# SMART-TTS/SMART-NAR_Fast_TTS

Measured on AMD Instinct MI355X. Metric: mel_frames_per_sec, higher is better.
Workload: dtype f32

## Files before the change

### include/nar_fs2.h

```cpp
#ifndef NAR_FS2_H
#define NAR_FS2_H

#include <stddef.h>
#include <stdint.h>

#ifdef __cplusplus
extern "C" {
#endif

#define NS_ABI_VERSION 6

typedef struct ns_model ns_model;

typedef struct ns_config {
  int32_t n_vocab;
  int32_t max_seq_len;
  int32_t d_enc, n_enc_layer, n_enc_head;
  int32_t d_dec, n_dec_layer, n_dec_head;
  int32_t d_inner;
  int32_t ffn_k1, ffn_k2;
  int32_t vp_filter, vp_kernel;
  int32_t n_bins;
  int32_t n_mel;
  int32_t postnet_dim, postnet_k, postnet_n;
// ... 37 lines not shown
                                 size_t ws_aln_bytes, float* log_d, uint8_t* src_mask, int64_t* mel_lens, float* p_pred, float* e_pred,
                                 float* tgt_output, float* attn_all_layers, int64_t* d_targets, void* stream);
int ns_upload_lengths(const int64_t* host, int n, int64_t* dev, void* stream);

#define NS_STATUS_TRUNCATED 1
#define NS_STATUS_BAD_TOKEN 2
int ns_forward_mel(ns_model* m, int B, int L, int T, const int64_t* mel_lens, float p_control, float e_control,
                   const float* p_targets, const float* e_targets, const void* ws_enc, void* ws_dec, size_t ws_dec_bytes,
                   float* mel, float* postnet_mel, float* p_pred, float* e_pred, uint8_t* mel_mask, int32_t* status, void* stream);

int ns_forward_mel_packed(ns_model* m, int B, int L, int T, const int64_t* mel_lens, const int64_t* mel_lens_host,
                          float p_control, float e_control, const float* p_targets, const float* e_targets, const void* ws_enc,
                          void* ws_dec, size_t ws_dec_bytes, float* mel, float* postnet_mel, float* p_pred, float* e_pred,
                          uint8_t* mel_mask, int32_t* status, void* stream);
int64_t ns_last_phase2_rows(const ns_model* m);

size_t ns_op_ws_bytes(const ns_model* m, int B, int S);
int ns_op_mask_from_lengths(const int64_t* lens, int B, int max_len, uint8_t* mask, void* stream);
int ns_op_sinusoid_table(int n_position, int d_hid, float* out, void* stream);
int ns_op_txt_encoder(ns_model* m, const int64_t* texts, const int64_t* lens, int B, int L, float* out, void* ws, size_t ws_bytes, void* stream);
int ns_op_multi_head_attention(ns_model* m, const char* prefix, const float* x, const int64_t* lens, int B, int S, float* out, void* ws, size_t ws_bytes, void* stream);
int ns_op_positionwise_ffn(ns_model* m, const char* prefix, const float* x, int B, int S, float* out, void* ws, size_t ws_bytes, void* stream);
int ns_op_fft_block(ns_model* m, const char* prefix, const float* x, const int64_t* lens, int B, int S, float* out, void* ws, size_t ws_bytes, void* stream);
int ns_op_variance_predictor(ns_model* m, const char* prefix, const float* x, const int64_t* lens, int B, int S, float* out, void* ws, size_t ws_bytes, void* stream);
int ns_op_predictor_conv1(ns_model* m, const char* prefix, const float* x, int B, int S, float* h, void* ws, size_t ws_bytes, void* stream);
int ns_op_predictor_tail(ns_model* m, const char* prefix, const float* h, const int64_t* lens, int B, int S, float control,
                         const float* target , const float* x_in , int add_pos, float* pred,
                         float* x_out , void* ws, size_t ws_bytes, void* stream);
int ns_op_duration_round(const float* log_d, int n, float d_control, float* d_rounded, void* stream);
int ns_op_duration_scan(const float* d_rounded, int B, int L, int32_t* cum, int64_t* mel_lens, void* stream);
// ... 312 lines not shown
```

### smart-nar_fast_tts_amd/_lib.py

```python
from __future__ import annotations

import ctypes as C
import os

import torch

_HERE = os.path.dirname(os.path.abspath(__file__))
LIB_PATH = os.path.join(_HERE, "csrc", "libnarfs2.so")


class NsConfig(C.Structure):
    _fields_ = [(n, C.c_int32) for n in (
        "n_vocab", "max_seq_len", "d_enc", "n_enc_layer", "n_enc_head", "d_dec", "n_dec_layer", "n_dec_head",
        "d_inner", "ffn_k1", "ffn_k2", "vp_filter", "vp_kernel", "n_bins", "n_mel",
        "postnet_dim", "postnet_k", "postnet_n", "pitch_frame_level", "energy_frame_level", "length_regulator",
        "matmul_bf16x3", "row_epilogue", "phase1_packing")]


class NsLossArgs(C.Structure):
    _fields_ = ([(n, C.c_int32) for n in ("B", "L", "T", "H", "n_mel", "pitch_frame_level", "energy_frame_level")]
                + [(n, C.c_int64) for n in ("mel_targets_stride", "d_targets_stride")]
                + [(n, C.c_void_p) for n in ("mel", "postnet", "mel_targets", "mel_masks", "pitch", "pitch_targets", "energy", "energy_targets",
                                             "log_d", "d_targets", "src_masks", "src_lens", "mel_lens")]
                + [("attn", C.c_void_p * 4)])
# ... 39 lines not shown
class NsPgWeights(C.Structure):
    _fields_ = [(n, C.c_void_p) for n in PG_NAMES]


class NsPgGrads(C.Structure):
    _fields_ = [(n, C.c_void_p) for n in PG_NAMES + ("dx",)]


class NsMelConfig(C.Structure):
    _fields_ = [(n, C.c_int32) for n in ("filter_length", "hop_length", "win_length", "n_mel")] + [("clip_val", C.c_float)]


class NsGlConfig(C.Structure):
    _fields_ = [(n, C.c_int32) for n in ("filter_length", "hop_length", "win_length", "n_mel")] + [("spec_from_mel_scaling", C.c_float)]


_P, _I, _F, _Z, _S = C.c_void_p, C.c_int, C.c_float, C.c_size_t, C.c_char_p

SIGNATURES = {
    "ns_last_error": (C.c_char_p, []),
    "ns_create": (_I, [C.POINTER(NsConfig), C.POINTER(_P)]),
    "ns_destroy": (None, [_P]),
    "ns_arena_bytes": (_Z, [_P]),
    "ns_bind_arena": (_I, [_P, _P, _Z]),
    "ns_set_weight": (_I, [_P, _S, _P, C.POINTER(C.c_int64), _I]),
    "ns_check_weight": (_I, [_P, _S, C.POINTER(C.c_int64), _I]),
    "ns_finalize_weights": (_I, [_P, _P]),
    "ns_adopt_arena": (_I, [_P]),
    "ns_encoder_ws_bytes": (_Z, [_P, _I, _I]),
    "ns_decoder_ws_bytes": (_Z, [_P, _I, _I, _I]),
    "ns_forward_durations": (_I, [_P, _P, _P, _I, _I, _F, _F, _F, _P, _P, _P, _Z, _P, _P, _P, _P, _P, _P, _P, _P]),
    "ns_forward_durations_packed": (_I, [_P, _P, _P, _P, _I, _I, _F, _F, _F, _P, _P, _P, _Z, _P, _P, _P, _P, _P, _P, _P, _P]),
    "ns_forward_durations_teacher": (_I, [_P, _P, _P, _P, _P, _P, _I, _I, _I, _F, _F, _P, _P, _P, _Z, _P, _Z, _P, _P, _P, _P, _P, _P, _P, _P, _P]),
    "ns_last_phase1_rows": (C.c_int64, [_P]),
    "ns_upload_lengths": (_I, [_P, _I, _P, _P]),
    "ns_forward_mel": (_I, [_P, _I, _I, _I, _P, _F, _F, _P, _P, _P, _P, _Z, _P, _P, _P, _P, _P, _P, _P]),
    "ns_forward_mel_packed": (_I, [_P, _I, _I, _I, _P, _P, _F, _F, _P, _P, _P, _P, _Z, _P, _P, _P, _P, _P, _P, _P]),

    "ns_last_phase2_rows": (C.c_int64, [_P]),
    "ns_plan_gemm": (_I, [_I, _I, _I, _I, C.POINTER(C.c_int32)]),
    "ns_plan_gemm_launches": (_I, [_I, _I, _I, _I, _I, C.POINTER(C.c_int32)]),
    "ns_plan_row_tile": (_I, [_I, _I]),
    "ns_plan_row_tile_k": (_I, [_I, _I, _I]),
    "ns_acc_chunk": (_I, []),
    "ns_abi_version": (_I, []),
    "ns_plan_attention_split": (_I, [_I, _I, _I, _I]),
    "ns_op_ws_bytes": (_Z, [_P, _I, _I]),
    "ns_op_mask_from_lengths": (_I, [_P, _I, _I, _P, _P]),
    "ns_op_sinusoid_table": (_I, [_I, _I, _P, _P]),
    "ns_op_txt_encoder": (_I, [_P, _P, _P, _I, _I, _P, _P, _Z, _P]),
    "ns_op_multi_head_attention": (_I, [_P, _S, _P, _P, _I, _I, _P, _P, _Z, _P]),
    "ns_op_positionwise_ffn": (_I, [_P, _S, _P, _I, _I, _P, _P, _Z, _P]),
    "ns_op_fft_block": (_I, [_P, _S, _P, _P, _I, _I, _P, _P, _Z, _P]),
    "ns_op_variance_predictor": (_I, [_P, _S, _P, _P, _I, _I, _P, _P, _Z, _P]),
# ... 166 lines not shown
```

### smart-nar_fast_tts_amd/csrc/api.hip

```cpp
#include <cstdio>

#include "../../include/nar_fs2.h"
#include "host_core.h"

using namespace ns;

static thread_local std::string g_err;
static int fail(const std::string& s) { g_err = s; return 1; }

namespace {

struct LayerW { ConvW qkv, fc, w1, w2; size_t ln1_g, ln1_b, ln2_g, ln2_b; };
struct PredW { ConvW c1, c2; size_t ln1_g, ln1_b, ln2_g, ln2_b, lin_w, lin_b; };

}

struct ns_model {
  ns_config cfg;
  std::vector<LayerW> enc, dec;
  PredW pred[3];
  size_t hdr;
  size_t emb, enc_pos, dec_pos, pitch_bins, energy_bins, pitch_emb, energy_emb;
  ConvW mel_linear;
  size_t pn_in, pn_hid, pn_const;
  size_t pos_long;
  std::vector<ConvW> post;
  Arena ar;
  float* arena = nullptr;
  bool ready = false;
  WeightRegistry weights;
  const float* P(size_t off) const { return arena + off; }
  const unsigned short* plane(size_t off) const { return off != NO_PLANE ? reinterpret_cast<const unsigned short*>(P(off)) : nullptr; }
  ConvGemm conv(const ConvW& w) const {
// ... 151 lines not shown
    ConvW w = m->ar.conv(cout, c.postnet_k, cin);
    if (c.matmul_bf16x3 == 1 && cin == c.postnet_dim && cout == c.postnet_dim) take_b3(m->ar, w);
    if (c.matmul_bf16x3 == 2) take_bf(m->ar, w);
    m->post.push_back(w);
  }
  m->pn_in = m->ar.take((size_t)PN_CONST_ROWS * c.n_mel);
  m->pn_hid = m->ar.take((size_t)2 * PN_CONST_ROWS * c.postnet_dim);
  m->pn_const = m->ar.take((size_t)PN_CONST_ROWS * c.n_mel);
  m->pos_long = m->ar.take((size_t)POS_LONG_ROWS * c.d_dec);
  *out = m;
  return 0;
}

extern "C" void ns_destroy(ns_model* m) {
  if (!m) return;
  for (auto& ps : m->prof_slot)
    for (auto& ev : ps.ev) { (void)hipEventDestroy(ev.first); (void)hipEventDestroy(ev.second); }
  delete m;
}
extern "C" size_t ns_arena_bytes(const ns_model* m) { return m ? m->ar.n * sizeof(float) : 0; }

extern "C" int ns_bind_arena(ns_model* m, void* dev, size_t bytes) { return bind_arena(m, dev, bytes, ns_arena_bytes(m), "ns_bind_arena"); }

extern "C" int ns_adopt_arena(ns_model* m) {
  if (!m || !m->arena) return fail("ns_adopt_arena: no arena bound");
  uint32_t got[ARENA_HDR_WORDS], want[ARENA_HDR_WORDS];
  int cur_dev = 0;
  NS_HIP(hipGetDevice(&cur_dev));
  hipPointerAttribute_t at;
  NS_HIP(hipPointerGetAttributes(&at, m->arena));
// ... 103 lines not shown
  NS_HIP(launch_sinusoid(POS_LONG_ROWS, c.d_dec, m->arena + m->pos_long, st));
  NS_HIP(hipStreamSynchronize(st));
  m->weights.release();
  m->ready = true;
  return 0;
}

namespace {
struct PackedCtx { RowMap rm; int Mp; };

struct Scratch {
  const PackedCtx* pk;
  float *xa, *xb, *qkv, *att, *t1, *x1, *hid, *vp1, *vp2, *pos_ext, *att_part;
  size_t att_part_floats;
  Tickets tk;
};

static size_t imax(size_t a, size_t b) { return a > b ? a : b; }

static Scratch carve(const ns_config& c, Bump& bp, size_t M, int S, bool no_split = false) {
  Scratch s;
  s.pk = nullptr;
  const size_t d = c.d_enc;
  s.xa = bp.f(M * d); s.xb = bp.f(M * d);
  s.qkv = bp.f(M * 3 * d); s.att = bp.f(M * d); s.t1 = bp.f(M * d); s.x1 = bp.f(M * d);
  s.hid = bp.f(M * imax(c.d_inner, 2 * (size_t)c.postnet_dim));
  s.vp1 = bp.f(M * c.vp_filter); s.vp2 = bp.f(M * c.vp_filter);
  s.pos_ext = S > c.max_seq_len ? bp.f((size_t)S * d) : nullptr;
  const int hmax = c.n_enc_head > c.n_dec_head ? c.n_enc_head : c.n_dec_head;
  int nsp = 1;
// ... 244 lines not shown
  sc.hid = m->arena + m->pn_hid;
  return postnet(m, in, 1, PN_CONST_ROWS, in, m->arena + m->pn_const, sc, st);
}

static int encoder(ns_model* m, const long long* texts, const long long* lens, int B, int L, float* out, Scratch& sc,
                   hipStream_t st) {
  const ns_config& c = m->cfg;
  const int M = rows_of(sc, B, L), d = c.d_enc;
  const float* pos;
  NS_TRY(position_rows(m, m->enc_pos, L, d, sc, &pos, st));
  float* cur = m->enc.empty() ? out : sc.xa;
  if (sc.pk) NS_HIP(launch_embed_pos_packed(texts, m->P(m->emb), pos, cur, sc.pk->rm, B, M, L, d, c.n_vocab, sc.tk.base, TICKET_INTS, st));
  else NS_HIP(launch_embed_pos(texts, m->P(m->emb), pos, cur, M, L, d, c.n_vocab, sc.tk.base, TICKET_INTS, st));
  for (size_t i = 0; i < m->enc.size(); ++i) {
    float* dst = (i + 1 == m->enc.size()) ? out : (cur == sc.xa ? sc.xb : sc.xa);
    NS_TRY(fft_block(m, m->enc[i], d, c.n_enc_head, cur, lens, B, L, dst, sc, st));
    cur = dst;
  }
  return 0;
}

static int decoder_stack(ns_model* m, float* x, const long long* lens, int B, int T, float* out, Scratch& sc, hipStream_t st) {
  const ns_config& c = m->cfg;
  float* cur = x;
  float* alt = (x == sc.xa) ? sc.xb : sc.xa;
  for (size_t i = 0; i < m->dec.size(); ++i) {
    float* dst = (i + 1 == m->dec.size()) ? out : alt;
    NS_TRY(fft_block(m, m->dec[i], c.d_dec, c.n_dec_head, cur, lens, B, T, dst, sc, st));
    if (dst != out) { alt = cur; cur = dst; }
  }
// ... 30 lines not shown
  ns_aligner* aln;
  const float* mels;
  const int64_t* mel_lens_in;
  int T;
  void* ws_aln;
  size_t ws_aln_bytes;
  float *tgt_output, *attn;
  int64_t* d_targets;
};

static int forward_durations(ns_model* m, const int64_t* texts, const int64_t* src_lens, const int64_t* lens_host, int B, int L, float d_control,
                             float p_control, float e_control, const float* p_targets, const float* e_targets,
                             void* ws_enc, size_t ws_bytes, float* log_d, float* d_rounded, uint8_t* src_mask,
                             int64_t* mel_lens, float* p_pred, float* e_pred, int64_t* mel_lens_host, void* stream,
                             const Teacher* tf = nullptr) {
  NS_TRY(check_ready(m));
  if (B <= 0 || L <= 0) return fail("ns_forward_durations: empty batch");
  if (ws_bytes < ns_encoder_ws_bytes(m, B, L)) return fail("ns_forward_durations: workspace too small");
  hipStream_t st = (hipStream_t)stream;
  const ns_config& c = m->cfg;
  if (!c.pitch_frame_level && !p_pred) return fail("ns_forward_durations: phoneme_level pitch needs a p_pred [B,L] output");
  if (!c.energy_frame_level && !e_pred) return fail("ns_forward_durations: phoneme_level energy needs an e_pred [B,L] output");
  Bump bp(ws_enc);
  float* enc_out = bp.f((size_t)B * L * c.d_enc);
  int32_t* cum = (int32_t*)bp.raw((size_t)B * L * sizeof(int32_t));
  float* dur_keep = bp.f((size_t)B * L);
  const long long* lens = (const long long*)src_lens;
  size_t Mp = 0;
  bool packed = lens_host && !m->enc.empty() && launch_planner_enabled() && c.pitch_frame_level && c.energy_frame_level && c.phase1_packing != 2;
  if (packed) {
    Mp = phase1_packed_rows(lens_host, B, L);
    auto cu_rows = [&](size_t rows) {
      const size_t ntn = (size_t)c.d_inner / 128, w32 = (rows + 31) / 32 * ntn, w48 = (rows + 47) / 48 * ntn;
      return (conv_gemm_tile16_enabled() && w32 > 256 && w48 <= 256) ? (size_t)48 : 32 * ((w32 + 255) / 256);
    };
    packed = Mp > 0 && Mp * 10 <= (size_t)B * L * 9 && (c.phase1_packing == 1 || cu_rows(Mp) < cu_rows((size_t)B * L));
  }
  const size_t Mrows = packed ? Mp : (size_t)B * L;
  m->last_rows1 = (long long)Mrows;
  Scratch sc = carve(c, bp, Mrows, L, packed);
  PackedCtx pk;
  memset(&pk, 0, sizeof(pk));
  float *enc_w = enc_out, *logd_w = log_d;
  if (packed) {
    const int M = (int)Mp, d = c.d_enc;
    const int base = window_att_wgs(lens_host, B, L, PHONEME_GUARD, c.n_enc_head);
    size_t n = (size_t)attention_split_packed(base, L, d / c.n_enc_head, Mp, d);
    const size_t per = Mp * d + 2 * Mp * c.n_enc_head;
    const size_t extra = phase1_packed_extra_bytes(c, B, L);
    const size_t avail = ws_bytes > bp.off + extra ? (ws_bytes - bp.off - extra) / sizeof(float) : 0;
    while (n > 1 && n * per > avail) --n;
    if (n > 1) { sc.att_part_floats = n * per; sc.att_part = bp.f(sc.att_part_floats); }
    int* plan = (int*)bp.raw(pack_plan_ints(B, Mp) * sizeof(int));
    enc_w = bp.f(Mp * d); logd_w = bp.f(Mp);
    if (bp.off > ws_bytes) return fail("ns_forward_durations: workspace too small (packed rows)");
    pk.Mp = M;
    pk.rm.rows = M;
    pk.rm.att_wgs = base;
    NS_HIP(launch_pack_plan_only(lens, B, L, c.n_enc_head, M, plan, &pk.rm, st, PHONEME_GUARD));
  }
  {
    sc.pk = packed ? &pk : nullptr;
    NS_TRY(encoder(m, (const long long*)texts, lens, B, L, enc_w, sc, st));
    if (tf) {
      if (tf->T > 0) NS_TRY(ns_aln_forward(tf->aln, enc_w, src_lens, tf->mels, tf->mel_lens_in, B, L, tf->T, tf->tgt_output, tf->attn, tf->d_targets,
                                           tf->ws_aln, tf->ws_aln_bytes, stream));
      else NS_HIP(hipMemsetAsync(tf->d_targets, 0, (size_t)B * L * sizeof(int64_t), st));
    }
    NS_TRY(predictor(m, m->pred[0], enc_w, lens, B, L, 1.0f, nullptr, logd_w, nullptr, nullptr, nullptr, nullptr, sc, st));
    if (!c.pitch_frame_level)
      NS_TRY(predictor(m, m->pred[1], enc_w, lens, B, L, p_control, p_targets, p_pred, m->P(m->pitch_bins), m->P(m->pitch_emb), nullptr, enc_w, sc, st));
    if (!c.energy_frame_level)
      NS_TRY(predictor(m, m->pred[2], enc_w, lens, B, L, e_control, e_targets, e_pred, m->P(m->energy_bins), m->P(m->energy_emb), nullptr, enc_w, sc, st));
  }
  if (packed) {
    NS_HIP(launch_unpack_phase1(pk.rm, lens, B, L, c.d_enc, enc_w, enc_out, logd_w, log_d, st));
  }
  if (tf) {
    NS_HIP(launch_duration_target_tail((const long long*)tf->d_targets, lens, (const long long*)texts, c.n_vocab, B, L, dur_keep, cum,
                                       (long long*)mel_lens, src_mask, st));
    return 0;
  }
  NS_HIP(launch_duration_tail(log_d, lens, (const long long*)texts, c.n_vocab, B, L, d_control, d_rounded, dur_keep, cum,
// ... 115 lines not shown
      NS_HIP(launch_pack_plan(lens, B, T, c.n_dec_head, M, plan, &pk.rm, st));
      NS_HIP(launch_gaussian_upsampling(enc_out, dur_keep, B, L, c.d_enc, T, T, sc.xa, sc.vp2, nullptr, lens, status, sc.tk.base, TICKET_INTS, st, &pk.rm));
    } else {
      NS_HIP(launch_length_regulate_packed(enc_out, cum, B, L, c.d_enc, T, M, c.n_dec_head, sc.xa, lens, status, sc.tk.base, TICKET_INTS, plan, &pk.rm, st));
    }
    pk.rm.att_wgs = window_att_wgs(lens_host, B, T, PACK_GUARD, c.n_dec_head);
    if (p_targets && c.pitch_frame_level) { NS_HIP(launch_pack_vector(pk.rm, T, p_targets, pt_p, M, st)); p_targets = pt_p; }
    if (e_targets && c.energy_frame_level) { NS_HIP(launch_pack_vector(pk.rm, T, e_targets, et_p, M, st)); e_targets = et_p; }
  } else if (c.length_regulator == 1) {
    NS_HIP(launch_mask_from_lengths(lens, B, T, mel_mask, st));
    if ((size_t)B * (L + 1) > (size_t)M * c.vp_filter) return fail("ns_forward_mel: workspace too small for the Gaussian centres");
    NS_HIP(launch_gaussian_upsampling(enc_out, dur_keep, B, L, c.d_enc, T, T, sc.xa, sc.vp2, nullptr, lens, status, sc.tk.base, TICKET_INTS, st));
  } else {
    NS_HIP(launch_length_regulate(enc_out, cum, B, L, c.d_enc, T, sc.xa, mel_mask, lens, status, sc.tk.base, TICKET_INTS, st));
  }
  sc.pk = packed ? &pk : nullptr;
  float* const mel_dst = packed ? mel_p : mel;
  float* const post_dst = packed ? post_p : postnet_mel;
  float* const pp_dst = packed ? pp_p : p_pred;
  float* const ep_dst = packed ? ep_p : e_pred;
  const float* pos;
  NS_TRY(position_rows(m, m->dec_pos, T, d, sc, &pos, st));
  float* cur = sc.xa;
  float* alt = sc.xb;
  if (c.pitch_frame_level) {
    if (!p_pred) return fail("ns_forward_mel: frame_level pitch needs a p_pred [B,T] output");
    NS_TRY(predictor(m, m->pred[1], cur, lens, B, T, p_control, p_targets, pp_dst, m->P(m->pitch_bins), m->P(m->pitch_emb),
                     c.energy_frame_level ? nullptr : pos, alt, sc, st));
    float* t = cur; cur = alt; alt = t;
  }
// ... 27 lines not shown
extern "C" int ns_forward_mel(ns_model* m, int B, int L, int T, const int64_t* mel_lens, float p_control, float e_control,
                              const float* p_targets, const float* e_targets,
                              const void* ws_enc, void* ws_dec, size_t ws_bytes, float* mel, float* postnet_mel, float* p_pred,
                              float* e_pred, uint8_t* mel_mask, int32_t* status, void* stream) {
  return forward_mel(m, B, L, T, mel_lens, nullptr, p_control, e_control, p_targets, e_targets, ws_enc, ws_dec, ws_bytes, mel, postnet_mel,
                     p_pred, e_pred, mel_mask, status, stream);
}

extern "C" int ns_forward_mel_packed(ns_model* m, int B, int L, int T, const int64_t* mel_lens, const int64_t* mel_lens_host,
                                     float p_control, float e_control, const float* p_targets, const float* e_targets,
                                     const void* ws_enc, void* ws_dec, size_t ws_bytes, float* mel, float* postnet_mel, float* p_pred,
                                     float* e_pred, uint8_t* mel_mask, int32_t* status, void* stream) {
  if (!mel_lens_host) return fail("ns_forward_mel_packed: mel_lens_host (the host copy of mel_lens) is required");
  return forward_mel(m, B, L, T, mel_lens, mel_lens_host, p_control, e_control, p_targets, e_targets, ws_enc, ws_dec, ws_bytes, mel,
                     postnet_mel, p_pred, e_pred, mel_mask, status, stream);
}

static int find_layer(ns_model* m, const char* prefix_c, const LayerW** L, int* d, int* H, const char* suffix) {
  std::string p(prefix_c ? prefix_c : "");
  if (suffix && *suffix) {
    if (!ends_with(p, suffix)) return fail("prefix '" + p + "' does not end with '" + suffix + "'");
    p.resize(p.size() - strlen(suffix));
  }
  const bool enc = starts_with(p, "txt_encoder.layer_stack."), dec = starts_with(p, "mel_decoder.layer_stack.");
  if (!enc && !dec) return fail("unknown module prefix '" + std::string(prefix_c ? prefix_c : "") + "'");
  const char* num = p.c_str() + (enc ? strlen("txt_encoder.layer_stack.") : strlen("mel_decoder.layer_stack."));
  char* end = nullptr;
  const long idx = strtol(num, &end, 10);
  if (end == num || *end != 0 || *num < '0' || *num > '9') return fail("no layer index in '" + std::string(prefix_c ? prefix_c : "") + "'");
  auto& v = enc ? m->enc : m->dec;
// ... 450 lines not shown
```

### smart-nar_fast_tts_amd/model.py

```python
from __future__ import annotations

import builtins
import contextlib
import ctypes as C
import functools
import json
import math
import os
import time
from collections import OrderedDict
from typing import NamedTuple

import numpy as np
import torch

from . import _lib
from . import workload as wl


def config_struct(preprocess_config: dict, model_config: dict) -> _lib.NsConfig:
    t = model_config["transformer"]
    vp = model_config["variance_predictor"]
    pp = preprocess_config["preprocessing"]
    for lvl in (pp["pitch"]["feature"], pp["energy"]["feature"]):
# ... 34 lines not shown
        off, n, shape, dtype = self.at[name]
        return self.buf[off:off + n].view(dtype).view(shape)


_ITEMSIZE = {torch.float32: 4, torch.bool: 1, torch.long: 8, torch.int32: 4}


@functools.lru_cache(maxsize=2048)
def _block_layout(specs):
    off, at = 0, {}
    for name, shape, dtype in specs:
        n = math.prod(shape) * _ITEMSIZE[dtype]
        at[name] = (off, n, shape, dtype)
        off += (n + _OutputBlock._ALIGN - 1) // _OutputBlock._ALIGN * _OutputBlock._ALIGN
    return at, max(off, _OutputBlock._ALIGN)


class ForwardOutput(tuple):

    def __new__(cls, items, status=None, n_vocab=0):
        self = super().__new__(cls, items)
        self.status = status
        self._n_vocab = n_vocab
        return self

    def check(self):
        if self.status is None:
            return []
        words = self.status.cpu().tolist()
        bad = [i for i, w in enumerate(words) if w & _lib.STATUS_BAD_TOKEN]
# ... 401 lines not shown
            last_use[k[1]] = i
        for old in sorted(last_use, key=last_use.get)[:max(0, len(last_use) - max_streams)]:
            for k in [k for k in ws if k[1] == old]:
                del ws[k]

    def _pinned_lens(self, B: int, stream_handle=None):
        key = ("pin", stream_handle if stream_handle is not None else torch.cuda.current_stream(self._device).cuda_stream)
        t = self._ws.get(key)
        if t is None or t[0].numel() < B:
            buf = torch.empty(max(B, 64), dtype=torch.long, pin_memory=True)
            t = (buf, buf.numpy())
            self._ws[key] = t
        self._ws.move_to_end(key)
        return t[0][:B], t[1][:B]

    def _device_lens(self, B: int, stream_handle) -> torch.Tensor:
        key = ("lens", stream_handle)
        t = self._ws.get(key)
        if t is None or t.numel() < B:
            t = torch.empty(max(B, 64), dtype=torch.long, device=self._device)
            self._ws[key] = t
        self._ws.move_to_end(key)
        return t[:B]

    def _ws_bytes(self, kind: str, B: int, L: int, T: int) -> int:
        key = (kind, B, L, T)
        n = self._ws_need.get(key)
        if n is None:
            n = (self._lib.ns_encoder_ws_bytes(self._h, B, L) if kind == "enc" else self._lib.ns_decoder_ws_bytes(self._h, B, L, T))
            if len(self._ws_need) > 4096:
                self._ws_need.clear()
            self._ws_need[key] = n
        return n

    def release_workspaces(self):
        self._ws = OrderedDict()

    def __call__(self, *args, **kwargs):
        return self.forward(*args, **kwargs)

    SPIN_US = builtins.float(os.environ.get("NS_SPIN_US", "300"))

    _UNWRITTEN = int(np.iinfo(np.int64).min)
    POLL_PINNED = os.environ.get("NS_POLL_PINNED", "1") != "0"

    def _wait_phase1(self, dev, pin_np=None):
        if self.SPIN_US > 0:
            deadline = time.perf_counter() + self.SPIN_US * 1e-6
            if pin_np is not None and self.POLL_PINNED:
                while int(pin_np.min()) == self._UNWRITTEN:
                    if time.perf_counter() > deadline:
                        break
                else:
                    return
            else:
                done = torch.cuda.Event()
                done.record(torch.cuda.current_stream(dev))
                while not done.query():
                    if time.perf_counter() > deadline:
# ... 68 lines not shown
            if not p_frame:
                o1.append(("p_pred", (B, L), f32))
            if not e_frame:
                o1.append(("e_pred", (B, L), f32))
            blk1 = _OutputBlock(o1, dev)
            ws_enc = self._workspace("enc", self._ws_bytes("enc", B, L, 0), sh)
            fixed_T = isinstance(max_mel_len, (int, np.integer)) and not isinstance(max_mel_len, bool)
            if async_status and not fixed_T:
                raise ValueError("async_status=True needs max_mel_len=<int>: without a host read the mel axis must be fixed by the caller")
            if fixed_T and int(max_mel_len) < 0:
                raise ValueError(f"max_mel_len ({int(max_mel_len)}) is negative")
            pin = pin_np = None
            if not (fixed_T and async_status):
                pin, pin_np = self._pinned_lens(B, sh)
                pin_np.fill(self._UNWRITTEN)
            tail1 = (B, L, 1.0, float(p_control), float(e_control),
                     _lib.ptr(None if p_frame else target("p_targets", p_targets, (B, L))),
                     _lib.ptr(None if e_frame else target("e_targets", e_targets, (B, L))),
                     _lib.ptr(ws_enc), ws_enc.numel(), blk1.ptr("log_d"), blk1.ptr("d_rounded"), blk1.ptr("src_masks"),
                     blk1.ptr("mel_lens"), blk1.ptr("p_pred"), blk1.ptr("e_pred"), _lib.ptr(pin), st)
            if lens_host is not None and self.packed_rows:
                _lib.check(lib.ns_forward_durations_packed(self._h, _lib.ptr(texts_c), _lib.ptr(lens_c), C.c_void_p(lens_host.ctypes.data), *tail1),
                           "ns_forward_durations_packed")
            else:
                _lib.check(lib.ns_forward_durations(self._h, _lib.ptr(texts_c), _lib.ptr(lens_c), *tail1), "ns_forward_durations")
            blk2 = ws_dec = None
            lens_on_host = False
            if fixed_T and async_status:
                T = int(max_mel_len)
            else:
                hint = int(max_mel_len) if fixed_T else self._t_hint.get((B, L))
                if hint is not None and p_targets is None and e_targets is None:
                    Tc = hint if fixed_T else hint + max(8, hint >> 3)
                    blk2 = _OutputBlock(phase2_outputs(Tc), dev)
                    ws_dec = self._workspace("dec", self._ws_bytes("dec", B, L, Tc), sh)
                self._wait_phase1(dev, pin_np)
                lens_on_host = True
                T = int(pin_np.max())
                if int(pin_np.min()) < 0:
                    bad = [i for i, v in enumerate(pin_np.tolist()) if v < 0]
                    raise IndexError(f"index out of range in self: token id outside [0, {self._cfg.n_vocab}) in utterance(s) {bad}")
                if fixed_T:
                    if int(max_mel_len) < T:
                        cut = [i for i, v in enumerate(pin_np.tolist()) if v > int(max_mel_len)]
                        raise ValueError(f"max_mel_len ({int(max_mel_len)}) is smaller than the longest utterance ({T}): utterance(s) {cut}")
                    T = int(max_mel_len)
                elif callable(max_mel_len):
                    longest = T
                    T = int(max_mel_len(torch.tensor(longest, device=dev)))
                    if T < longest:
                        raise ValueError(f"max_mel_len() returned {T}, smaller than the longest utterance ({longest})")
                else:
                    if len(self._t_hint) > 4096:
                        self._t_hint.clear()
                    self._t_hint[(B, L)] = T
                if blk2 is not None and T > Tc:
                    blk2 = ws_dec = None
            if blk2 is None:
                blk2 = _OutputBlock(phase2_outputs(T), dev)
                ws_dec = self._workspace("dec", self._ws_bytes("dec", B, L, max(T, 1)), sh)
            else:
                blk2.layout(phase2_outputs(T))
                need = self._ws_bytes("dec", B, L, max(T, 1))
                if ws_dec.numel() < need:
                    ws_dec = self._workspace("dec", need, sh)
            tg0 = target("p_targets", p_targets, (B, T)) if p_frame else None
            tg1 = target("e_targets", e_targets, (B, T)) if e_frame else None
            tail = (float(p_control), float(e_control), _lib.ptr(tg0), _lib.ptr(tg1), _lib.ptr(ws_enc), _lib.ptr(ws_dec), ws_dec.numel(),
                    blk2.ptr("mel"), blk2.ptr("post"), blk2.ptr("p_pred") if p_frame else None,
                    blk2.ptr("e_pred") if e_frame else None, blk2.ptr("mel_masks"), blk1.ptr("status"), st)
            if lens_on_host and self.packed_rows:
                _lib.check(lib.ns_forward_mel_packed(self._h, B, L, T, blk1.ptr("mel_lens"), _lib.ptr(pin), *tail), "ns_forward_mel_packed")
            else:
                _lib.check(lib.ns_forward_mel(self._h, B, L, T, blk1.ptr("mel_lens"), *tail), "ns_forward_mel")
            log_d, d_rounded, src_masks = blk1.view("log_d"), blk1.view("d_rounded"), blk1.view("src_masks")
            out_mel_lens, status = blk1.view("mel_lens"), blk1.view("status")
            mel, post, mel_masks = blk2.view("mel"), blk2.view("post"), blk2.view("mel_masks")
            p_pred = blk2.view("p_pred") if p_frame else blk1.view("p_pred")
            e_pred = blk2.view("e_pred") if e_frame else blk1.view("e_pred")
        items = (mel, post, p_pred, e_pred, log_d, d_rounded, src_masks, mel_masks, src_lens, out_mel_lens, None, None)
        if self.outputs == "separate":
            with torch.cuda.stream(torch.cuda.current_stream(dev)):
                items = tuple(t.clone() if (torch.is_tensor(t) and i != 8) else t for i, t in enumerate(items))
                status = status.clone()
        out = ForwardOutput(items, status=status, n_vocab=self._cfg.n_vocab)
        self._last_out = ForwardOutput((), status=status, n_vocab=self._cfg.n_vocab)
# ... 86 lines not shown
```

Baseline: 2.946 million.

## Move phase-1 to phase-2 handover into native code with mid-encoder event wait

Adds a native handover path that waits for the host copy of mel lengths, picks T and the output block layout, and enqueues the mel decoder in one C call. This removes the Python-side wait, layout and launch overhead between the two phases. It also records an event before the last encoder layer (or before the predictors) so the host can block instead of spinning through the long part of phase 1, then spin only near the end. The cost is more code paths, duplicated layout logic that must match the Python one, and a new arm/handle state machine.

```diff
diff --git a/include/nar_fs2.h b/include/nar_fs2.h
--- a/include/nar_fs2.h
+++ b/include/nar_fs2.h
@@ -75,6 +75,36 @@
                           void* ws_dec, size_t ws_dec_bytes, float* mel, float* postnet_mel, float* p_pred, float* e_pred,
                           uint8_t* mel_mask, int32_t* status, void* stream);
 int64_t ns_last_phase2_rows(const ns_model* m);
+
+#define NS_HO_ABI_VERSION 1
+#define NS_HO_OUTPUTS 5
+#define NS_HO_LAUNCHED 0
+#define NS_HO_BAD_TOKEN 1
+#define NS_HO_NO_FIT 2
+#define NS_HO_FIXED_T 1
+#define NS_HO_PACKED 2
+#define NS_HO_TIMES 7
+typedef struct ns_handover ns_handover;
+typedef struct ns_handover_plan {
+  int32_t code;
+  int32_t T;
+  int32_t longest;
+  int32_t n_bad;
+  int64_t offset[NS_HO_OUTPUTS];
+  int64_t nbytes;
+  int64_t ws_need;
+} ns_handover_plan;
+int ns_ho_abi_version(void);
+int64_t ns_phase2_layout(int B, int T, int n_mel, int pitch_frame_level, int energy_frame_level, int64_t offset[NS_HO_OUTPUTS]);
+int ns_handover_decide(const ns_model* m, const int64_t* lens, int B, int L, int t_cap, int flags, size_t block_bytes, size_t ws_dec_bytes,
+                       ns_handover_plan* plan, int32_t* bad_idx);
+int ns_handover_create(ns_model* m, void* stream, ns_handover** out);
+void ns_handover_destroy(ns_handover* h);
+int ns_handover_arm(ns_model* m, ns_handover* h);
+int ns_forward_handover(ns_model* m, ns_handover* h, int B, int L, int t_cap, int flags, double spin_us, const int64_t* mel_lens,
+                        const int64_t* mel_lens_host, float p_control, float e_control, const void* ws_enc, void* ws_dec,
+                        size_t ws_dec_bytes, void* block, size_t block_bytes, int32_t* status, void* stream, ns_handover_plan* plan,
+                        int32_t* bad_idx, double* times_us);
 
 size_t ns_op_ws_bytes(const ns_model* m, int B, int S);
 int ns_op_mask_from_lengths(const int64_t* lens, int B, int max_len, uint8_t* mask, void* stream);
diff --git a/smart-nar_fast_tts_amd/_lib.py b/smart-nar_fast_tts_amd/_lib.py
--- a/smart-nar_fast_tts_amd/_lib.py
+++ b/smart-nar_fast_tts_amd/_lib.py
@@ -77,6 +77,15 @@
 class NsGlConfig(C.Structure):
     _fields_ = [(n, C.c_int32) for n in ("filter_length", "hop_length", "win_length", "n_mel")] + [("spec_from_mel_scaling", C.c_float)]
 
+
+class NsHandoverPlan(C.Structure):
+    _fields_ = ([(n, C.c_int32) for n in ("code", "T", "longest", "n_bad")] + [("offset", C.c_int64 * 5), ("nbytes", C.c_int64), ("ws_need", C.c_int64)])
+
+
+HO_LAUNCHED, HO_BAD_TOKEN, HO_NO_FIT = 0, 1, 2
+HO_FIXED_T, HO_PACKED = 1, 2
+HO_OUTPUTS = ("mel", "post", "mel_masks", "p_pred", "e_pred")
+HO_TIMES = ("spin", "sleep", "second spin", "block", "C after the wait", "first launch", "phase-2 enqueue")
 
 _P, _I, _F, _Z, _S = C.c_void_p, C.c_int, C.c_float, C.c_size_t, C.c_char_p
 
@@ -101,6 +110,14 @@
     "ns_forward_mel_packed": (_I, [_P, _I, _I, _I, _P, _P, _F, _F, _P, _P, _P, _P, _Z, _P, _P, _P, _P, _P, _P, _P]),
 
     "ns_last_phase2_rows": (C.c_int64, [_P]),
+    "ns_ho_abi_version": (_I, []),
+    "ns_phase2_layout": (C.c_int64, [_I, _I, _I, _I, _I, C.POINTER(C.c_int64)]),
+    "ns_handover_decide": (_I, [_P, _P, _I, _I, _I, _I, _Z, _Z, C.POINTER(NsHandoverPlan), C.POINTER(C.c_int32)]),
+    "ns_handover_create": (_I, [_P, _P, C.POINTER(_P)]),
+    "ns_handover_destroy": (None, [_P]),
+    "ns_handover_arm": (_I, [_P, _P]),
+    "ns_forward_handover": (_I, [_P, _P, _I, _I, _I, _I, C.c_double, _P, _P, _F, _F, _P, _P, _Z, _P, _Z, _P, _P, C.POINTER(NsHandoverPlan),
+                                C.POINTER(C.c_int32), C.POINTER(C.c_double)]),
     "ns_plan_gemm": (_I, [_I, _I, _I, _I, C.POINTER(C.c_int32)]),
     "ns_plan_gemm_launches": (_I, [_I, _I, _I, _I, _I, C.POINTER(C.c_int32)]),
     "ns_plan_row_tile": (_I, [_I, _I]),
diff --git a/smart-nar_fast_tts_amd/csrc/api.hip b/smart-nar_fast_tts_amd/csrc/api.hip
--- a/smart-nar_fast_tts_amd/csrc/api.hip
+++ b/smart-nar_fast_tts_amd/csrc/api.hip
@@ -2,6 +2,9 @@
 
 #include "../../include/nar_fs2.h"
 #include "host_core.h"
+#include "handover_core.h"
+
+#include <chrono>
 
 using namespace ns;
 
@@ -15,8 +18,18 @@
 
 }
 
+struct ns_handover {
+  ns_model* m;
+  hipStream_t stream;
+  hipEvent_t mid, done;
+  bool mid_recorded;
+};
+
 struct ns_model {
   ns_config cfg;
+  std::vector<ns_handover*> handovers;
+  ns_handover* armed = nullptr;
+  std::chrono::steady_clock::time_point* first_launch = nullptr;
   std::vector<LayerW> enc, dec;
   PredW pred[3];
   size_t hdr;
@@ -198,6 +211,7 @@
 
 extern "C" void ns_destroy(ns_model* m) {
   if (!m) return;
+  for (ns_handover* h : m->handovers) h->m = nullptr;
   for (auto& ps : m->prof_slot)
     for (auto& ev : ps.ev) { (void)hipEventDestroy(ev.first); (void)hipEventDestroy(ev.second); }
   delete m;
@@ -331,6 +345,7 @@
   float *xa, *xb, *qkv, *att, *t1, *x1, *hid, *vp1, *vp2, *pos_ext, *att_part;
   size_t att_part_floats;
   Tickets tk;
+  ns_handover* mid = nullptr;
 };
 
 static size_t imax(size_t a, size_t b) { return a > b ? a : b; }
@@ -605,6 +620,7 @@
   else NS_HIP(launch_embed_pos(texts, m->P(m->emb), pos, cur, M, L, d, c.n_vocab, sc.tk.base, TICKET_INTS, st));
   for (size_t i = 0; i < m->enc.size(); ++i) {
     float* dst = (i + 1 == m->enc.size()) ? out : (cur == sc.xa ? sc.xb : sc.xa);
+    if (i + 1 == m->enc.size() && sc.mid) { NS_HIP(hipEventRecord(sc.mid->mid, st)); sc.mid->mid_recorded = true; sc.mid = nullptr; }
     NS_TRY(fft_block(m, m->enc[i], d, c.n_enc_head, cur, lens, B, L, dst, sc, st));
     cur = dst;
   }
@@ -665,6 +681,8 @@
                              void* ws_enc, size_t ws_bytes, float* log_d, float* d_rounded, uint8_t* src_mask,
                              int64_t* mel_lens, float* p_pred, float* e_pred, int64_t* mel_lens_host, void* stream,
                              const Teacher* tf = nullptr) {
+  ns_handover* const armed = m ? m->armed : nullptr;
+  if (m) m->armed = nullptr;
   NS_TRY(check_ready(m));
   if (B <= 0 || L <= 0) return fail("ns_forward_durations: empty batch");
   if (ws_bytes < ns_encoder_ws_bytes(m, B, L)) return fail("ns_forward_durations: workspace too small");
@@ -690,6 +708,7 @@
   const size_t Mrows = packed ? Mp : (size_t)B * L;
   m->last_rows1 = (long long)Mrows;
   Scratch sc = carve(c, bp, Mrows, L, packed);
+  sc.mid = (armed && !tf && armed->stream == st) ? armed : nullptr;
   PackedCtx pk;
   memset(&pk, 0, sizeof(pk));
   float *enc_w = enc_out, *logd_w = log_d;
@@ -718,6 +737,7 @@
                                            tf->ws_aln, tf->ws_aln_bytes, stream));
       else NS_HIP(hipMemsetAsync(tf->d_targets, 0, (size_t)B * L * sizeof(int64_t), st));
     }
+    if (sc.mid) { NS_HIP(hipEventRecord(sc.mid->mid, st)); sc.mid->mid_recorded = true; sc.mid = nullptr; }
     NS_TRY(predictor(m, m->pred[0], enc_w, lens, B, L, 1.0f, nullptr, logd_w, nullptr, nullptr, nullptr, nullptr, sc, st));
     if (!c.pitch_frame_level)
       NS_TRY(predictor(m, m->pred[1], enc_w, lens, B, L, p_control, p_targets, p_pred, m->P(m->pitch_bins), m->P(m->pitch_emb), nullptr, enc_w, sc, st));
@@ -863,6 +883,7 @@
   } else {
     NS_HIP(launch_length_regulate(enc_out, cum, B, L, c.d_enc, T, sc.xa, mel_mask, lens, status, sc.tk.base, TICKET_INTS, st));
   }
+  if (m->first_launch) { *m->first_launch = std::chrono::steady_clock::now(); m->first_launch = nullptr; }
   sc.pk = packed ? &pk : nullptr;
   float* const mel_dst = packed ? mel_p : mel;
   float* const post_dst = packed ? post_p : postnet_mel;
@@ -920,6 +941,147 @@
   if (!mel_lens_host) return fail("ns_forward_mel_packed: mel_lens_host (the host copy of mel_lens) is required");
   return forward_mel(m, B, L, T, mel_lens, mel_lens_host, p_control, e_control, p_targets, e_targets, ws_enc, ws_dec, ws_bytes, mel,
                      postnet_mel, p_pred, e_pred, mel_mask, status, stream);
+}
+
+extern "C" int ns_ho_abi_version(void) { return NS_HO_ABI_VERSION; }
+
+extern "C" int64_t ns_phase2_layout(int B, int T, int n_mel, int pitch_frame_level, int energy_frame_level, int64_t offset[NS_HO_OUTPUTS]) {
+  int64_t dummy[NS_HO_OUTPUTS];
+  return ns_ho_layout(B, T, n_mel, pitch_frame_level, energy_frame_level, offset ? offset : dummy);
+}
+
+namespace {
+struct WsRule { const ns_model* m; int B, L; };
+static size_t decoder_ws_rule(const void* ctx, int T) {
+  const WsRule* r = (const WsRule*)ctx;
+  return ns_decoder_ws_bytes(r->m, r->B, r->L, T);
+}
+}
+
+extern "C" int ns_handover_decide(const ns_model* m, const int64_t* lens, int B, int L, int t_cap, int flags, size_t block_bytes,
+                                  size_t ws_dec_bytes, ns_handover_plan* plan, int32_t* bad_idx) {
+  if (!m || !lens || !plan) return fail("ns_handover_decide: null argument");
+  if (B <= 0 || L <= 0) return fail("ns_handover_decide: empty batch");
+  if (t_cap < 0) return fail("ns_handover_decide: negative capacity");
+  const WsRule rule = {m, B, L};
+  ns_ho_decide(lens, B, t_cap, flags, m->cfg.n_mel, m->cfg.pitch_frame_level, m->cfg.energy_frame_level, block_bytes, ws_dec_bytes,
+               decoder_ws_rule, &rule, plan, bad_idx);
+  return 0;
+}
+
+extern "C" int ns_handover_create(ns_model* m, void* stream, ns_handover** out) {
+  if (!m || !out) return fail("ns_handover_create: null argument");
+  ns_handover* h = new ns_handover{m, (hipStream_t)stream, nullptr, nullptr, false};
+  hipError_t e = hipEventCreateWithFlags(&h->mid, hipEventDisableTiming | hipEventBlockingSync);
+  if (e == hipSuccess) e = hipEventCreateWithFlags(&h->done, hipEventDisableTiming | hipEventBlockingSync);
+  if (e != hipSuccess) {
+    if (h->mid) (void)hipEventDestroy(h->mid);
+    delete h;
+    return fail(std::string("ns_handover_create: ") + hipGetErrorString(e));
+  }
+  m->handovers.push_back(h);
+  *out = h;
+  return 0;
+}
+
+extern "C" void ns_handover_destroy(ns_handover* h) {
+  if (!h) return;
+  if (h->m) {
+    if (h->m->armed == h) h->m->armed = nullptr;
+    auto& v = h->m->handovers;
+    for (size_t i = 0; i < v.size(); ++i)
+      if (v[i] == h) { v.erase(v.begin() + i); break; }
+  }
+  (void)hipEventDestroy(h->mid);
+  (void)hipEventDestroy(h->done);
+  delete h;
+}
+
+extern "C" int ns_handover_arm(ns_model* m, ns_handover* h) {
+  if (!m || !h || h->m != m) return fail("ns_handover_arm: the handle belongs to another model");
+  h->mid_recorded = false;
+  m->armed = h;
+  return 0;
+}
+
+namespace {
+using HoClock = std::chrono::steady_clock;
+static double us_since(HoClock::time_point t0) { return std::chrono::duration<double, std::micro>(HoClock::now() - t0).count(); }
+static bool lens_written(const int64_t* pin, int B) {
+  for (int b = 0; b < B; ++b)
+    if (__atomic_load_n(&pin[b], __ATOMIC_ACQUIRE) == INT64_MIN) return false;
+  return true;
+}
+static bool spin_for(const int64_t* pin, int B, double budget_us) {
+  if (lens_written(pin, B)) return true;
+  if (!(budget_us > 0)) return false;
+  const HoClock::time_point t0 = HoClock::now();
+  do {
+    for (int i = 0; i < 16; ++i) {
+#if defined(__x86_64__)
+      __asm__ __volatile__("pause" ::: "memory");
+#endif
+      if (lens_written(pin, B)) return true;
+    }
+  } while (us_since(t0) < budget_us);
+  return lens_written(pin, B);
+}
+}
+
+extern "C" int ns_forward_handover(ns_model* m, ns_handover* h, int B, int L, int t_cap, int flags, double spin_us, const int64_t* mel_lens,
+                                   const int64_t* mel_lens_host, float p_control, float e_control, const void* ws_enc, void* ws_dec,
+                                   size_t ws_dec_bytes, void* block, size_t block_bytes, int32_t* status, void* stream, ns_handover_plan* plan,
+                                   int32_t* bad_idx, double* times_us) {
+  NS_TRY(check_ready(m));
+  if (!h || h->m != m) return fail("ns_forward_handover: the handle belongs to another model");
+  if (!mel_lens || !mel_lens_host || !ws_enc || !ws_dec || !block || !status || !plan) return fail("ns_forward_handover: null argument");
+  if (B <= 0 || L <= 0) return fail("ns_forward_handover: empty batch");
+  if (t_cap < 0) return fail("ns_forward_handover: negative capacity");
+  if ((uintptr_t)block & (NS_HO_ALIGN - 1)) return fail("ns_forward_handover: the output block must be 256-byte aligned");
+  hipStream_t st = (hipStream_t)stream;
+  if (h->stream != st) return fail("ns_forward_handover: the handle was created for another stream");
+  double tm[NS_HO_TIMES] = {0, 0, 0, 0, 0, 0, 0};
+  HoClock::time_point t0 = HoClock::now();
+  bool ready = spin_for(mel_lens_host, B, spin_us);
+  tm[0] = us_since(t0);
+  const bool stretch = h->mid_recorded;
+  h->mid_recorded = false;
+  if (!ready && stretch) {
+    t0 = HoClock::now();
+    NS_HIP(hipEventSynchronize(h->mid));
+    tm[1] = us_since(t0);
+    t0 = HoClock::now();
+    ready = spin_for(mel_lens_host, B, spin_us);
+    tm[2] = us_since(t0);
+  }
+  if (!ready) {
+    t0 = HoClock::now();
+    NS_HIP(hipEventRecord(h->done, st));
+    NS_HIP(hipEventSynchronize(h->done));
+    tm[3] = us_since(t0);
+    if (!lens_written(mel_lens_host, B)) return fail("ns_forward_handover: phase 1 completed without writing mel_lens_host");
+  }
+  t0 = HoClock::now();
+  std::vector<int64_t> lens((size_t)B);
+  for (int b = 0; b < B; ++b) lens[b] = __atomic_load_n(&mel_lens_host[b], __ATOMIC_RELAXED);
+  NS_TRY(ns_handover_decide(m, lens.data(), B, L, t_cap, flags, block_bytes, ws_dec_bytes, plan, bad_idx));
+  tm[4] = us_since(t0);
+  int rc = 0;
+  if (plan->code == NS_HO_LAUNCHED) {
+    t0 = HoClock::now();
+    HoClock::time_point first = t0;
+    m->first_launch = times_us ? &first : nullptr;
+    char* const base = (char*)block;
+    auto at = [&](int i) { return plan->offset[i] >= 0 ? base + plan->offset[i] : nullptr; };
+    rc = forward_mel(m, B, L, plan->T, mel_lens, (flags & NS_HO_PACKED) ? lens.data() : nullptr, p_control, e_control, nullptr, nullptr, ws_enc,
+                     ws_dec, ws_dec_bytes, (float*)at(0), (float*)at(1), (float*)at(3), (float*)at(4), (uint8_t*)at(2), status, stream);
+    m->first_launch = nullptr;
+    tm[5] = std::chrono::duration<double, std::micro>(first - t0).count();
+    tm[6] = us_since(t0);
+  }
+  if (times_us)
+    for (int i = 0; i < NS_HO_TIMES; ++i) times_us[i] = tm[i];
+  return rc;
 }
 
 static int find_layer(ns_model* m, const char* prefix_c, const LayerW** L, int* d, int* H, const char* suffix) {
diff --git a/smart-nar_fast_tts_amd/csrc/handover_core.h b/smart-nar_fast_tts_amd/csrc/handover_core.h
--- /dev/null
+++ b/smart-nar_fast_tts_amd/csrc/handover_core.h
@@ -0,0 +1,57 @@
+#ifndef NS_HANDOVER_CORE_H
+#define NS_HANDOVER_CORE_H
+
+#include <stddef.h>
+#include <stdint.h>
+
+#define NS_HO_ALIGN 256
+
+typedef size_t (*ns_ho_ws_rule)(const void* ctx, int T);
+
+static inline int64_t ns_ho_take(int64_t* off, int64_t bytes) {
+  const int64_t at = *off;
+  *off += (bytes + NS_HO_ALIGN - 1) / NS_HO_ALIGN * NS_HO_ALIGN;
+  return at;
+}
+
+static inline int64_t ns_ho_layout(int B, int T, int n_mel, int pitch_frame_level, int energy_frame_level, int64_t offset[NS_HO_OUTPUTS]) {
+  const int64_t rows = (int64_t)(B > 0 ? B : 0) * (T > 0 ? T : 0);
+  int64_t off = 0;
+  offset[0] = ns_ho_take(&off, rows * n_mel * 4);
+  offset[1] = ns_ho_take(&off, rows * n_mel * 4);
+  offset[2] = ns_ho_take(&off, rows);
+  offset[3] = pitch_frame_level ? ns_ho_take(&off, rows * 4) : -1;
+  offset[4] = energy_frame_level ? ns_ho_take(&off, rows * 4) : -1;
+  return off > NS_HO_ALIGN ? off : NS_HO_ALIGN;
+}
+
+static inline void ns_ho_decide(const int64_t* lens, int B, int t_cap, int flags, int n_mel, int pitch_frame_level, int energy_frame_level,
+                                size_t block_bytes, size_t ws_bytes, ns_ho_ws_rule rule, const void* ctx, ns_handover_plan* plan,
+                                int32_t* bad_idx) {
+  int64_t longest = 0;
+  int b, i, n_bad = 0;
+  for (b = 0; b < B; ++b) {
+    if (lens[b] < 0) {
+      if (bad_idx) bad_idx[n_bad] = b;
+      ++n_bad;
+    } else if (lens[b] > longest) {
+      longest = lens[b];
+    }
+  }
+  plan->n_bad = n_bad;
+  plan->longest = longest > INT32_MAX ? INT32_MAX : (int32_t)longest;
+  plan->T = 0;
+  plan->nbytes = 0;
+  plan->ws_need = 0;
+  for (i = 0; i < NS_HO_OUTPUTS; ++i) plan->offset[i] = -1;
+  if (n_bad) { plan->code = NS_HO_BAD_TOKEN; return; }
+  plan->code = NS_HO_NO_FIT;
+  if (longest > (int64_t)t_cap) return;
+  plan->T = (flags & NS_HO_FIXED_T) ? t_cap : (int32_t)longest;
+  plan->nbytes = ns_ho_layout(B, plan->T, n_mel, pitch_frame_level, energy_frame_level, plan->offset);
+  plan->ws_need = (int64_t)rule(ctx, plan->T > 0 ? plan->T : 1);
+  if ((uint64_t)plan->nbytes > (uint64_t)block_bytes || (uint64_t)plan->ws_need > (uint64_t)ws_bytes) return;
+  plan->code = NS_HO_LAUNCHED;
+}
+
+#endif
diff --git a/smart-nar_fast_tts_amd/model.py b/smart-nar_fast_tts_amd/model.py
--- a/smart-nar_fast_tts_amd/model.py
+++ b/smart-nar_fast_tts_amd/model.py
@@ -72,6 +72,45 @@
         at[name] = (off, n, shape, dtype)
         off += (n + _OutputBlock._ALIGN - 1) // _OutputBlock._ALIGN * _OutputBlock._ALIGN
     return at, max(off, _OutputBlock._ALIGN)
+
+
+def native_block_layout(lib, B, T, n_mel, p_frame, e_frame, offsets=None):
+    if offsets is None:
+        offsets = (C.c_int64 * len(_lib.HO_OUTPUTS))()
+        nbytes = int(lib.ns_phase2_layout(B, T, n_mel, int(p_frame), int(e_frame), offsets))
+    else:
+        nbytes = None
+    at = {}
+    for name, off in zip(_lib.HO_OUTPUTS, offsets):
+        if off >= 0:
+            shape, dtype = ((B, T), torch.bool) if name == "mel_masks" else ((B, T), torch.float32) if name.endswith("_pred") else ((B, T, n_mel), torch.float32)
+            at[name] = (int(off), math.prod(shape) * _ITEMSIZE[dtype], shape, dtype)
+    return at, nbytes
+
+
+class _Handover:
+
+    def __init__(self, lib, model_handle, stream_handle):
+        self._lib = lib
+        self.h = C.c_void_p()
+        _lib.check(lib.ns_handover_create(model_handle, C.c_void_p(stream_handle), C.byref(self.h)), "ns_handover_create")
+        self.plan = _lib.NsHandoverPlan()
+        self.plan_ref = C.byref(self.plan)
+        self.bad = (C.c_int32 * 64)()
+        self.times = (C.c_double * len(_lib.HO_TIMES))()
+
+    def bad_idx(self, B):
+        if len(self.bad) < B:
+            self.bad = (C.c_int32 * B)()
+        return self.bad
+
+    def __del__(self):
+        try:
+            if self.h:
+                self._lib.ns_handover_destroy(self.h)
+                self.h = None
+        except Exception:
+            pass
 
 
 class ForwardOutput(tuple):
@@ -503,6 +542,14 @@
         self._ws.move_to_end(key)
         return t[0][:B], t[1][:B]
 
+    def _handover(self, stream_handle) -> _Handover:
+        key = ("handover", stream_handle)
+        t = self._ws.get(key)
+        if t is None:
+            t = self._ws[key] = _Handover(self._lib, self._h, stream_handle)
+        self._ws.move_to_end(key)
+        return t
+
     def _device_lens(self, B: int, stream_handle) -> torch.Tensor:
         key = ("lens", stream_handle)
         t = self._ws.get(key)
@@ -532,6 +579,8 @@
 
     _UNWRITTEN = int(np.iinfo(np.int64).min)
     POLL_PINNED = os.environ.get("NS_POLL_PINNED", "1") != "0"
+
+    NATIVE_HANDOVER = True
 
     def _wait_phase1(self, dev, pin_np=None):
         if self.SPIN_US > 0:
@@ -630,6 +679,11 @@
             if not (fixed_T and async_status):
                 pin, pin_np = self._pinned_lens(B, sh)
                 pin_np.fill(self._UNWRITTEN)
+            ho = None
+            if (pin is not None and p_targets is None and e_targets is None and not callable(max_mel_len) and self.POLL_PINNED
+                    and (fixed_T or (B, L) in self._t_hint) and self.NATIVE_HANDOVER and os.environ.get("NS_NATIVE_HANDOVER", "1") != "0"):
+                ho = self._handover(sh)
+                _lib.check(lib.ns_handover_arm(self._h, ho.h), "ns_handover_arm")
             tail1 = (B, L, 1.0, float(p_control), float(e_control),
                      _lib.ptr(None if p_frame else target("p_targets", p_targets, (B, L))),
                      _lib.ptr(None if e_frame else target("e_targets", e_targets, (B, L))),
@@ -641,7 +695,7 @@
             else:
                 _lib.check(lib.ns_forward_durations(self._h, _lib.ptr(texts_c), _lib.ptr(lens_c), *tail1), "ns_forward_durations")
             blk2 = ws_dec = None
-            lens_on_host = False
+            lens_on_host = launched = False
             if fixed_T and async_status:
                 T = int(max_mel_len)
             else:
@@ -650,7 +704,18 @@
                     Tc = hint if fixed_T else hint + max(8, hint >> 3)
                     blk2 = _OutputBlock(phase2_outputs(Tc), dev)
                     ws_dec = self._workspace("dec", self._ws_bytes("dec", B, L, Tc), sh)
-                self._wait_phase1(dev, pin_np)
+                if ho is not None and blk2 is not None:
+                    plan = ho.plan
+                    _lib.check(lib.ns_forward_handover(
+                        self._h, ho.h, B, L, Tc, (_lib.HO_FIXED_T if fixed_T else 0) | (_lib.HO_PACKED if self.packed_rows else 0),
+                        self.SPIN_US, blk1.ptr("mel_lens"), _lib.ptr(pin), float(p_control), float(e_control), _lib.ptr(ws_enc), _lib.ptr(ws_dec),
+                        ws_dec.numel(), C.c_void_p(blk2.base), blk2.buf.numel(), blk1.ptr("status"), st, ho.plan_ref, ho.bad_idx(B), ho.times),
+                        "ns_forward_handover")
+                    launched = plan.code == _lib.HO_LAUNCHED
+                if launched:
+                    blk2.at, _ = native_block_layout(lib, B, plan.T, n_mel, p_frame, e_frame, plan.offset)
+                else:
+                    self._wait_phase1(dev, pin_np)
                 lens_on_host = True
                 T = int(pin_np.max())
                 if int(pin_np.min()) < 0:
@@ -672,7 +737,9 @@
                     self._t_hint[(B, L)] = T
                 if blk2 is not None and T > Tc:
                     blk2 = ws_dec = None
-            if blk2 is None:
+            if launched:
+                pass
+            elif blk2 is None:
                 blk2 = _OutputBlock(phase2_outputs(T), dev)
                 ws_dec = self._workspace("dec", self._ws_bytes("dec", B, L, max(T, 1)), sh)
             else:
@@ -685,7 +752,9 @@
             tail = (float(p_control), float(e_control), _lib.ptr(tg0), _lib.ptr(tg1), _lib.ptr(ws_enc), _lib.ptr(ws_dec), ws_dec.numel(),
                     blk2.ptr("mel"), blk2.ptr("post"), blk2.ptr("p_pred") if p_frame else None,
                     blk2.ptr("e_pred") if e_frame else None, blk2.ptr("mel_masks"), blk1.ptr("status"), st)
-            if lens_on_host and self.packed_rows:
+            if launched:
+                pass
+            elif lens_on_host and self.packed_rows:
                 _lib.check(lib.ns_forward_mel_packed(self._h, B, L, T, blk1.ptr("mel_lens"), _lib.ptr(pin), *tail), "ns_forward_mel_packed")
             else:
                 _lib.check(lib.ns_forward_mel(self._h, B, L, T, blk1.ptr("mel_lens"), *tail), "ns_forward_mel")
```

New measurement: 2.947 million, median of 2. About the same (+0.0%).
